# radiocosmology/draco

Measured on AMD Instinct MI355X. Metric: m-modes/sec through MModeTransform+DirtyMapMaker (128-feed, 256-freq), higher is better.
Workload: dtype f64 accumulate; B stored complex128; FFT complex64 (as the reference); 1 GPU; cfg3: 128-feed (379 stacked baselines), 256 freq per GPU (256 in the job), 1024 RA, lmax=mmax=512: MModeTransform.process + DirtyMapMaker.process through the task classes (131328 (m,f) solves + alm2map to nside=256 IQUV maps per GPU and day); parallelism=freq-sharded x1, weak scaling (no collective in the timed region)

## Files before the change

### draco_amd/csrc/sht.hip

```cpp
#include "sht_common.h"
#include "sht_legendre.h"
#include "sht_rings.h"

namespace {

int get_geom(dmm_ctx* ctx, int nside, int lmax, int mmax, ShtGeom* out) {
  const int64_t key = ((int64_t)nside << 40) | ((int64_t)lmax << 20) | (int64_t)mmax;
  auto it = ctx->sht.find(key);
  const int nring = 4 * nside - 1;
  const size_t nd = (size_t)3 * nring + (mmax + 1);
  const size_t bytes = nd * sizeof(double) + (size_t)nring * sizeof(int64_t) + (size_t)nring * sizeof(int);
  const size_t coef_ofs = (bytes + 63) / 64 * 64;
  const size_t coef_rows = (size_t)coef_row0(mmax + 1, lmax);
  int blue_rmax = 0;
  std::vector<int64_t> bf_off(1, 0);
  int64_t bf_total = 0;
  for (int ir = 1; ir < nside && blue_len(ir) <= kMaxBlue; ++ir) {
    bf_off.push_back(bf_total);
    bf_total += blue_len(ir);
    blue_rmax = ir;
  }
  const size_t bfo_ofs = coef_ofs + coef_rows * sizeof(Coef);
  const size_t bf_ofs = (bfo_ofs + bf_off.size() * sizeof(int64_t) + 63) / 64 * 64;
  const size_t phase_ofs = (bf_ofs + (size_t)bf_total * sizeof(double2) + 63) / 64 * 64;
// ... 86 lines not shown
  unsigned char* gb = static_cast<unsigned char*>(g.block);
  g.coef = reinterpret_cast<double*>(gb + coef_ofs);
  g.bf_off = reinterpret_cast<int64_t*>(gb + bfo_ofs);
  g.bfilt = reinterpret_cast<double2*>(gb + bf_ofs);
  g.blue_rmax = blue_rmax;
  g.phase = reinterpret_cast<double2*>(gb + phase_ofs);
  g.tw = reinterpret_cast<double2*>(gb + tw_ofs);
  g.tw_len = tw_len;
  g.chirp = reinterpret_cast<double2*>(gb + chirp_ofs);
  *out = g;
  return DMM_OK;
}

int check_args(const char* who, dmm_ctx* ctx, const void* a, const void* b, int nfreq, int npol, int lmax, int mmax,
               int nside) {
  DMM_REQUIRE(ctx && a && b, "%s: NULL argument", who);
  DMM_REQUIRE(nfreq >= 1 && lmax >= 0 && mmax >= 0 && mmax <= lmax, "%s: bad sizes nfreq=%d lmax=%d mmax=%d", who, nfreq, lmax, mmax);
  DMM_REQUIRE(npol == 1 || npol == 4, "%s: npol must be 1 or 4 (got %d)", who, npol);
  DMM_REQUIRE(nside >= 1 && (nside & (nside - 1)) == 0 && nside <= 8192, "%s: nside must be a power of two (got %d)", who, nside);
  return DMM_OK;
}

size_t chunk_freqs(int nfreq, int npol, int nring, int mmax) {
  const size_t per_f = (size_t)npol * nring * (mmax + 1) * sizeof(double2);
  size_t nf = ((size_t)1 << 30) / per_f;
  if (nf < 1) nf = 1;
  if (nf > (size_t)nfreq) nf = nfreq;
  const size_t nchunk = ((size_t)nfreq + nf - 1) / nf;
  return ((size_t)nfreq + nchunk - 1) / nchunk;
}

struct ClassLaunch {
  RingClass rc;
  int nblock;
  int nphi_max;
  bool blue;
};

std::vector<ClassLaunch> ring_classes(const ShtGeom& g) {
  std::vector<ClassLaunch> out;
  ClassLaunch b;
  b.rc.belt = 1;
  b.rc.r_lo = b.rc.r_hi = 0;
  b.rc.M = 4 * g.nside;
  b.rc.logM = 0;
  while ((1 << b.rc.logM) < b.rc.M) ++b.rc.logM;
  b.nblock = 2 * g.nside + 1;
  b.nphi_max = 4 * g.nside;
  b.blue = false;
  out.push_back(b);
  for (int ir = 1; ir < g.nside;) {
    const int M = blue_len(ir);
    int hi = ir;
    while (hi + 1 < g.nside && blue_len(hi + 1) == M) ++hi;
    ClassLaunch c;
    c.rc.belt = 0;
    c.rc.r_lo = ir;
    c.rc.r_hi = hi;
    c.rc.M = M;
    c.rc.logM = 0;
    while ((1 << c.rc.logM) < M) ++c.rc.logM;
    c.nblock = 2 * (hi - ir + 1);
    c.nphi_max = 4 * hi;
    c.blue = true;
    out.push_back(c);
    ir = hi + 1;
  }
  return out;
}

size_t ring_fft_lds(const ShtGeom& g, const ClassLaunch& c, int nrow, int force_direct, bool synth = false) {
  if (force_direct) return 0;
  if (c.blue && c.rc.r_hi > g.blue_rmax) return 0;
  const size_t rot = synth && c.blue && 4 * c.rc.r_lo < g.mmax + 1 ? (size_t)nrow * 2 * (g.mmax + 1) : 0;
  const size_t lds = ((size_t)nrow * (c.rc.M + 1) + c.rc.M / 2 + (c.blue ? c.nphi_max : 0) + rot) * sizeof(double2);
  return lds <= 160 * 1024 ? lds : 0;
}

template <typename K>
int launch_ring(K kern, dim3 grid, int threads, size_t lds, hipStream_t st, const RingParams& rp, const RingClass& rc) {
  if (lds > 160 * 1024) return dmm_set_error(DMM_E_UNSUPPORTED, "SHT ring stage needs %zu bytes of LDS (nside too large)", lds);
  DMM_HIP(hipFuncSetAttribute((const void*)kern, hipFuncAttributeMaxDynamicSharedMemorySize, (int)lds));
  hipLaunchKernelGGL(kern, grid, dim3(threads), lds, st, rp, rc);
  DMM_HIP(hipGetLastError());
  return DMM_OK;
}

template <int NPOL>
int synth_chunk(dmm_ctx* ctx, const ShtGeom& g, const double2* alm, int n_m, int nf, double2* b, double* map) {
  LegParams lp;
  lp.g = g;
  lp.nf = nf;
  lp.npol = NPOL;
  lp.n_m = n_m;
  lp.alm = alm;
  lp.b = b;
  lp.m_identity = (ctx->opt_sht_variant & 32) ? 1 : 0;
  if (NPOL == 4 && !(ctx->opt_sht_variant & 8)) {
    const int npair = (g.nring + 1) / 2;
    const int nrc = (npair + kThreads - 1) / kThreads;
#ifdef LEG_STAMPS
    static unsigned long long* stamps_d = nullptr;
    const size_t nst = (size_t)(g.mmax + 1) * nrc * ((nf + 2 * kLegF - 1) / (2 * kLegF)) * 4 * 8;
    if (!stamps_d) (void)hipMalloc((void**)&stamps_d, 64 << 20);
    (void)hipMemsetAsync(stamps_d, 0, nst * 8, ctx->stream);
    lp.stamps = stamps_d;
#endif
    const int nx = g.mmax + 1;
    const int64_t col_bytes = (int64_t)4 * n_m * (g.lmax + 1) * (int64_t)sizeof(double2);
    const bool fits8 = 2 * kLegF * col_bytes < ((int64_t)1 << 32), fits4 = kLegF * col_bytes < ((int64_t)1 << 32);
    if ((ctx->opt_sht_variant & 64) || ctx->opt_sht_synth_form == 1 || !fits4) {
      const int nz = (nf + kLegF - 1) / kLegF;
      hipLaunchKernelGGL(k_leg_synth_mfma, dim3(nx, nrc, nz), dim3(kThreads), 0, ctx->stream, lp);
    } else if ((ctx->opt_sht_variant & 128) || !fits8) {
      const int nz = (nf + kLegF - 1) / kLegF;
      hipLaunchKernelGGL(k_leg_synth_mfma2<1>, dim3(nx, nrc, nz), dim3(kThreads), 0, ctx->stream, lp);
    } else {
      const int nz = (nf + 2 * kLegF - 1) / (2 * kLegF);
      hipLaunchKernelGGL(k_leg_synth_mfma2<2>, dim3(nx, nrc, nz), dim3(kThreads), 0, ctx->stream, lp);
    }
  } else
  switch (ctx->opt_sht_variant & 3) {
    case 1: hipLaunchKernelGGL((k_leg_synth<NPOL, 1, 1>), dim3(g.mmax + 1, nf), dim3(kThreads), 0, ctx->stream, lp); break;
    case 2: hipLaunchKernelGGL((k_leg_synth<NPOL, 2, 1>), dim3(g.mmax + 1, nf), dim3(kThreads), 0, ctx->stream, lp); break;
    case 3: hipLaunchKernelGGL((k_leg_synth<NPOL, 1, 6>), dim3(g.mmax + 1, nf), dim3(kThreads), 0, ctx->stream, lp); break;
    default: hipLaunchKernelGGL((k_leg_synth<NPOL, 2, 4>), dim3(g.mmax + 1, nf), dim3(kThreads), 0, ctx->stream, lp); break;
  }
  DMM_HIP(hipGetLastError());
  RingParams rp;
  rp.g = g;
  rp.nf = nf;
  rp.npol = NPOL;
  rp.b = b;
  rp.map = map;
  rp.map_ref = nullptr;
  rp.radix8 = (ctx->opt_sht_variant & 2048) ? 0 : 1;
  rp.npix = 12LL * g.nside * g.nside;
  constexpr int NROWS = NPOL == 4 ? 2 : 1;
  const int force_direct = ctx->opt_sht_variant & 4;
  for (const ClassLaunch& c : ring_classes(g)) {
    const size_t lds2 = ring_fft_lds(g, c, NROWS, force_direct, true), lds1 = ring_fft_lds(g, c, 1, force_direct, true);
    int rc;
    if (lds1 == 0) {
      rc = launch_ring(k_ring_synth<NPOL>, dim3(c.nblock, nf), kThreads, (size_t)NPOL * (g.mmax + 1) * sizeof(double2), ctx->stream, rp, c.rc);
    } else if (NROWS == 2 && lds2 != 0 && lds2 <= 80 * 1024) {
      rc = c.blue ? launch_ring(k_ring_synth_fft<NPOL, NROWS, true>, dim3(c.nblock, nf), kFftThreads, lds2, ctx->stream, rp, c.rc)
                  : launch_ring(k_ring_synth_fft<NPOL, NROWS, false>, dim3(c.nblock, nf), kFftThreads, lds2, ctx->stream, rp, c.rc);
    } else {
      rc = c.blue ? launch_ring(k_ring_synth_fft<NPOL, 1, true>, dim3(c.nblock, nf, NROWS), kFftThreads, lds1, ctx->stream, rp, c.rc)
                  : launch_ring(k_ring_synth_fft<NPOL, 1, false>, dim3(c.nblock, nf, NROWS), kFftThreads, lds1, ctx->stream, rp, c.rc);
    }
    if (rc) return rc;
  }
  return DMM_OK;
}

template <int NPOL>
int anal_chunk(dmm_ctx* ctx, const ShtGeom& g, const double* map, int n_m, int nf, double2* b, double2* alm, int accumulate,
               const double* map_ref = nullptr) {
  RingParams rp;
  rp.g = g;
  rp.nf = nf;
  rp.npol = NPOL;
  rp.b = b;
  rp.map = const_cast<double*>(map);
  rp.map_ref = map_ref;
  rp.radix8 = (ctx->opt_sht_variant & 2048) ? 0 : 1;
  rp.npix = 12LL * g.nside * g.nside;
  constexpr int NROWS = NPOL == 4 ? 2 : 1;
  const int force_direct = ctx->opt_sht_variant & 4;
  for (const ClassLaunch& c : ring_classes(g)) {
    const size_t lds2 = ring_fft_lds(g, c, NROWS, force_direct), lds1 = ring_fft_lds(g, c, 1, force_direct);
    int rc;
    if (lds1 == 0) {
      rc = launch_ring(k_ring_anal<NPOL>, dim3(c.nblock, nf), kThreads, (size_t)NPOL * c.nphi_max * sizeof(double), ctx->stream, rp, c.rc);
    } else if (NROWS == 2 && lds2 != 0 && lds2 <= 80 * 1024) {
      rc = c.blue ? launch_ring(k_ring_anal_fft<NPOL, NROWS, true>, dim3(c.nblock, nf), kFftThreads, lds2, ctx->stream, rp, c.rc)
                  : launch_ring(k_ring_anal_fft<NPOL, NROWS, false>, dim3(c.nblock, nf), kFftThreads, lds2, ctx->stream, rp, c.rc);
    } else {
      rc = c.blue ? launch_ring(k_ring_anal_fft<NPOL, 1, true>, dim3(c.nblock, nf, NROWS), kFftThreads, lds1, ctx->stream, rp, c.rc)
                  : launch_ring(k_ring_anal_fft<NPOL, 1, false>, dim3(c.nblock, nf, NROWS), kFftThreads, lds1, ctx->stream, rp, c.rc);
    }
    if (rc) return rc;
  }
  LegAnalParams lp;
  lp.g = g;
  lp.nf = nf;
  lp.npol = NPOL;
  lp.n_m = n_m;
  lp.b = b;
  lp.alm = alm;
// ... 8 lines not shown
    return DMM_OK;
  }
  constexpr int NV = NPOL == 4 ? 8 : 2;
  const size_t lds2 = (size_t)(g.lmax + 1) * NV * sizeof(double) + (size_t)2 * (kThreads / 64) * kAnalBatch * NV * sizeof(double);
  DMM_HIP(hipFuncSetAttribute((const void*)k_leg_anal<NPOL>, hipFuncAttributeMaxDynamicSharedMemorySize, (int)lds2));
  hipLaunchKernelGGL(k_leg_anal<NPOL>, dim3(g.mmax + 1, nf), dim3(kThreads), lds2, ctx->stream, lp);
  DMM_HIP(hipGetLastError());
  return DMM_OK;
}

}

extern "C" {

int dmm_alm2map(dmm_ctx* ctx, const void* alm, int nfreq, int npol, int lmax, int mmax, int nside, double* map) {
  int rc = check_args("dmm_alm2map", ctx, alm, map, nfreq, npol, lmax, mmax, nside);
  if (rc) return rc;
  DMM_HIP(hipSetDevice(ctx->device));
  ShtGeom g;
  rc = get_geom(ctx, nside, lmax, mmax, &g);
  if (rc) return rc;
  const size_t nfc = chunk_freqs(nfreq, npol, g.nring, mmax);
  void* scratch = nullptr;
  rc = dmm_get_scratch(ctx, nfc * npol * g.nring * (size_t)(mmax + 1) * sizeof(double2), &scratch);
  if (rc) return rc;
  const int64_t npix = 12LL * nside * nside;
  const int n_m = mmax + 1;
  for (int f0 = 0; f0 < nfreq; f0 += (int)nfc) {
    const int nf = (int)((size_t)(nfreq - f0) < nfc ? (size_t)(nfreq - f0) : nfc);
    const double2* a = (const double2*)alm + (int64_t)f0 * npol * n_m * (lmax + 1);
    double* mp = map + (int64_t)f0 * npol * npix;
    rc = npol == 4 ? synth_chunk<4>(ctx, g, a, n_m, nf, (double2*)scratch, mp) : synth_chunk<1>(ctx, g, a, n_m, nf, (double2*)scratch, mp);
    if (rc) return rc;
  }
  return DMM_OK;
}

int dmm_map2alm(dmm_ctx* ctx, const double* map, int nfreq, int npol, int lmax, int mmax, int nside, int niter,
                void* alm) {
  int rc = check_args("dmm_map2alm", ctx, map, alm, nfreq, npol, lmax, mmax, nside);
  if (rc) return rc;
  DMM_REQUIRE(niter >= 0 && niter <= 64, "dmm_map2alm: niter=%d out of range", niter);
  if ((size_t)npol * 4 * nside * sizeof(double) > 150 * 1024)
    return dmm_set_error(DMM_E_UNSUPPORTED, "dmm_map2alm: nside=%d too large for the in-LDS ring stage", nside);
  DMM_HIP(hipSetDevice(ctx->device));
  ShtGeom g;
  rc = get_geom(ctx, nside, lmax, mmax, &g);
  if (rc) return rc;
  const int64_t npix = 12LL * nside * nside;
  size_t nfc = chunk_freqs(nfreq, npol, g.nring, mmax);
  const size_t b_bytes = nfc * npol * g.nring * (size_t)(mmax + 1) * sizeof(double2);
  const size_t r_bytes = niter > 0 ? nfc * npol * (size_t)npix * sizeof(double) : 0;
  void* scratch = nullptr;
  rc = dmm_get_scratch(ctx, b_bytes + r_bytes, &scratch);
  if (rc) return rc;
  double2* b = (double2*)scratch;
  double* resid = (double*)((unsigned char*)scratch + b_bytes);
  const int n_m = mmax + 1;
  for (int f0 = 0; f0 < nfreq; f0 += (int)nfc) {
    const int nf = (int)((size_t)(nfreq - f0) < nfc ? (size_t)(nfreq - f0) : nfc);
    double2* a = (double2*)alm + (int64_t)f0 * npol * n_m * (lmax + 1);
    const double* mp = map + (int64_t)f0 * npol * npix;
    rc = npol == 4 ? anal_chunk<4>(ctx, g, mp, n_m, nf, b, a, 0) : anal_chunk<1>(ctx, g, mp, n_m, nf, b, a, 0);
    if (rc) return rc;
    for (int it = 0; it < niter; ++it) {
      rc = npol == 4 ? synth_chunk<4>(ctx, g, a, n_m, nf, b, resid) : synth_chunk<1>(ctx, g, a, n_m, nf, b, resid);
      if (rc) return rc;
      rc = npol == 4 ? anal_chunk<4>(ctx, g, resid, n_m, nf, b, a, 1, mp) : anal_chunk<1>(ctx, g, resid, n_m, nf, b, a, 1, mp);
      if (rc) return rc;
    }
  }
  return DMM_OK;
}

// ... 2 lines not shown
```

### draco_amd/csrc/sht_common.h

```cpp
#pragma once
#include <math.h>

#include <vector>

#include "dmm_internal.h"
#include "fft_lds.h"

namespace {


constexpr int kThreads = 256;
constexpr double kBig = 0x1p+740, kSmallStep = 0x1p-800;

struct ShtGeom {
  int nside, lmax, mmax, nring;
  double* z;
  double* sth;
  double* phi0;
  int* nphi;
  int64_t* start;
  double* lfac;
  double* coef;
  double2* bfilt;
  int64_t* bf_off;
  int blue_rmax;
  double2* phase;
  double2* tw;
  int tw_len;
  double2* chirp;
  void* block;
};

__host__ __device__ __forceinline__ int64_t coef_row0(int m, int lmax) {
  return (int64_t)m * (lmax + 1) - (int64_t)m * (m - 1) / 2;
}

struct LegParams {
  ShtGeom g;
  int nf;
  int npol;
  int n_m;
  const double2* alm;
  double2* b;
  int m_identity;
#ifdef LEG_STAMPS
  unsigned long long* stamps;
#endif
};

struct Coef {
  double ra, rb;
  double c1, c2;
  double cd, c3;
  double c4, pad;
};

typedef const __attribute__((address_space(4))) double* kptr;

__device__ __forceinline__ Coef load_coef(kptr c) {
  Coef q;
  q.ra = c[0];
  q.rb = c[1];
  q.c1 = c[2];
  q.c2 = c[3];
  q.cd = c[4];
  q.c3 = c[5];
  q.c4 = c[6];
// ... 45 lines not shown
```

### draco_amd/csrc/sht_legendre.h

```cpp
#pragma once
#include "sht_common.h"

namespace {

__device__ __forceinline__ int leg_m_of_block(int b, int n_m, int variant_identity) {
  if (variant_identity) return b;
  const int q = b >> 6, r = b & 63;
  if (q * 64 + 64 > n_m) return b;
  return q * 64 + (r & 7) * 8 + (r >> 3);
}

template <int NPOL, int NR, int MINW>
__global__ __launch_bounds__(kThreads, MINW) void k_leg_synth(LegParams p) {
  const int m = blockIdx.x, f = blockIdx.y;
  const int lmax = p.g.lmax, nl = lmax - m + 1;
  const kptr coef = (kptr)p.g.coef + 8 * coef_row0(m, lmax);
  kptr a[NPOL];
#pragma unroll
  for (int q = 0; q < NPOL; ++q)
    a[q] = (kptr)(p.alm + (((int64_t)f * NPOL + q) * p.n_m + m) * (lmax + 1) + m);

  const int nring = p.g.nring, npair = (nring + 1) / 2;
  const double lfac_m = p.g.lfac[m];
  const int64_t mstride = p.g.mmax + 1;
  struct Ring {
    double x, inv_s2, xs2, lam, lam_prev;
    int nsc;
    double2 Ts, Ta, Vs, Va, Qs, Qa, Us, Ua;
  };
  for (int r0 = 0; r0 < npair; r0 += NR * kThreads) {
    Ring R[NR];
#pragma unroll
    for (int t = 0; t < NR; ++t) {
// ... 62 lines not shown
      if (NPOL == 4) {
        o.aE = load_c(a[NPOL > 1 ? 1 : 0] + 2 * kc);
        o.aB = load_c(a[NPOL > 1 ? 2 : 0] + 2 * kc);
        o.aV = load_c(a[NPOL > 1 ? 3 : 0] + 2 * kc);
      }
      return o;
    };
    Ops cur = fetch(0);
    for (int k = 0; k < nl; k += 2) {
      Ops nxt = fetch(k + 1);
#pragma unroll
      for (int t = 0; t < NR; ++t) step(R[t], cur.q, cur.aT, cur.aE, cur.aB, cur.aV, k == 0, true);
      if (k + 1 >= nl) break;
      cur = fetch(k + 2);
#pragma unroll
      for (int t = 0; t < NR; ++t) step(R[t], nxt.q, nxt.aT, nxt.aE, nxt.aB, nxt.aV, false, false);
    }
#pragma unroll
    for (int t = 0; t < NR; ++t) {
      const int r = r0 + t * kThreads + threadIdx.x;
      if (r >= npair) continue;
      const int rs = nring - 1 - r;
      const Ring& g = R[t];
      auto put = [&](int pol, int ring, double2 s, double2 an, double sgn) {
        p.b[(((int64_t)f * NPOL + pol) * nring + ring) * mstride + m] = make_double2(s.x + sgn * an.x, s.y + sgn * an.y);
      };
      put(0, r, g.Ts, g.Ta, 1.0);
      if (rs != r) put(0, rs, g.Ts, g.Ta, -1.0);
      if (NPOL == 4) {
        put(1, r, g.Qs, g.Qa, 1.0);
        put(2, r, g.Us, g.Ua, 1.0);
        put(3, r, g.Vs, g.Va, 1.0);
        if (rs != r) {
          put(1, rs, g.Qs, g.Qa, -1.0);
          put(2, rs, g.Us, g.Ua, -1.0);
          put(3, rs, g.Vs, g.Va, -1.0);
        }
      }
    }
  }
}

constexpr int kLegL = 8, kLegF = 4, kLegPitch = 72;

__device__ __forceinline__ void leg_synth_mfma_body(const LegParams& p, int bx, int by, int bz) {
  typedef double v4d __attribute__((ext_vector_type(4)));
  __shared__ double slab[kThreads / 64][3][kLegL][kLegPitch];
  const int m = leg_m_of_block(bx, p.g.mmax + 1, p.m_identity), rc = by, f0 = bz * kLegF;
  const int lmax = p.g.lmax, nl = lmax - m + 1;
  const int lane = threadIdx.x & 63, wave = threadIdx.x >> 6;
  const int nring = p.g.nring, npair = (nring + 1) / 2;
  const int64_t mstride = p.g.mmax + 1;
  double(*sl)[kLegL][kLegPitch] = slab[wave];

  const int r = rc * kThreads + threadIdx.x;
  double x = 0.0, inv_s2 = 0.0, xs2 = 0.0, lam = 0.0, lam_prev = 0.0;
  int nsc = -1;
  if (r < npair) {
    const double sth = p.g.sth[r];
    x = p.g.z[r];
    inv_s2 = 1.0 / (sth * sth);
    xs2 = x * inv_s2;
    if (!ring_skips_m(m, lmax, sth)) lam_start(p.g.lfac[m], m, sth, lam, nsc);
  }
  const bool wave_live = __any(nsc >= 0);

  const int li = lane & 15, kq = lane >> 4;
  const int col = li, fi = col >> 2, c = col & 3, f = f0 + fi;
  const bool fok = f < p.nf;
  auto colptr = [&](int pol, int comp) {
    return reinterpret_cast<const double*>(p.alm + (((int64_t)(fok ? f : 0) * 4 + pol) * p.n_m + m) * (lmax + 1) + m) + comp;
// ... 65 lines not shown
        sl[1][kk][lane] = F1;
        sl[2][kk][lane] = F2;
      }
      cv = cv_next;
#pragma unroll
      for (int par = 0; par < 2; ++par) {
        const bool ok = fok && c0 + 2 * kq + par < nl;
        const double bTV[2] = {ok ? rTV[0] : 0.0, ok ? rTV[1] : 0.0};
        const double b1[2] = {ok ? -r1[0] : 0.0, ok ? -r1[1] : 0.0};
        const double b2[2] = {ok ? s2 * r2[0] : 0.0, ok ? s2 * r2[1] : 0.0};
#pragma unroll
        for (int t = 0; t < 4; ++t) {
          const double aL = sl[0][2 * kq + par][16 * t + li];
          const double a1 = sl[1][2 * kq + par][16 * t + li];
          const double a2 = sl[2][2 * kq + par][16 * t + li];
          acc[t][par] = __builtin_amdgcn_mfma_f64_16x16x4f64(aL, bTV[par], acc[t][par], 0, 0, 0);
          acc[t][2 + par] = __builtin_amdgcn_mfma_f64_16x16x4f64(a1, b1[par], acc[t][2 + par], 0, 0, 0);
          acc[t][3 - par] = __builtin_amdgcn_mfma_f64_16x16x4f64(a2, b2[par], acc[t][3 - par], 0, 0, 0);
        }
      }
    }
  }
  if (!fok) return;
  double* bout = reinterpret_cast<double*>(p.b);
  const int comp = c & 1;
#pragma unroll
  for (int t = 0; t < 4; ++t)
#pragma unroll
    for (int reg = 0; reg < 4; ++reg) {
      const int rr = rc * kThreads + wave * 64 + 16 * t + kq + 4 * reg;
      if (rr >= npair) continue;
      const int rs = nring - 1 - rr;
#pragma unroll
      for (int g = 0; g < 2; ++g) {
        const int pol = g == 0 ? (c < 2 ? 0 : 3) : (c < 2 ? 1 : 2);
        const double sy = acc[t][2 * g][reg], an = acc[t][2 * g + 1][reg];
        bout[((((int64_t)f * 4 + pol) * nring + rr) * mstride + m) * 2 + comp] = sy + an;
        if (rs != rr) bout[((((int64_t)f * 4 + pol) * nring + rs) * mstride + m) * 2 + comp] = sy - an;
      }
    }
}

__global__ __launch_bounds__(kThreads, 2) void k_leg_synth_mfma(LegParams p) { leg_synth_mfma_body(p, blockIdx.x, blockIdx.y, blockIdx.z); }


constexpr int kLeg2Rows = kLegL + 1;
#ifndef PIPE_HINT
#define PIPE_HINT 1
#endif

template <int NFG>
__device__ __forceinline__ void leg_synth_mfma2_body(const LegParams& p, int bx, int by, int bz, int ny) {
  typedef double v4d __attribute__((ext_vector_type(4)));
  __shared__ double slab[kThreads / 64][2][kLeg2Rows][kLegPitch];
  __shared__ double ringf[kThreads / 64][2][64];
  const int m = leg_m_of_block(bx, p.g.mmax + 1, p.m_identity), rc = by, f0 = bz * (kLegF * NFG);
  const int lmax = p.g.lmax, nl = lmax - m + 1;
  const int lane = threadIdx.x & 63, wave = threadIdx.x >> 6;
  const int nring = p.g.nring, npair = (nring + 1) / 2;
  const int64_t mstride = p.g.mmax + 1;
  double(*sl)[kLeg2Rows][kLegPitch] = slab[wave];
#ifdef LEG_STAMPS
  unsigned long long st[6];
  auto stamp = [&](int i) {
    unsigned long long t;
    __builtin_amdgcn_sched_barrier(0);
    asm volatile("s_memrealtime %0\n\ts_waitcnt lgkmcnt(0)" : "=s"(t)::"memory");
    __builtin_amdgcn_sched_barrier(0);
    st[i] = t;
  };
  stamp(0);
#define LEG_STAMP(i) stamp(i)
#else
#define LEG_STAMP(i)
#endif

  const int NW = ny * (kThreads / 64), W = rc * (kThreads / 64) + wave;
  const int r = 16 * (W + (lane >> 4) * NW) + (lane & 15);
  double x = 0.0, lam = 0.0, lam_prev = 0.0;
// ... 164 lines not shown
      prep_load(nb, 0, 0);
      cvr = cvr_next;
      finish_ops(ops_next, c0n, ragged);
      ops = ops_next;
    };
    LEG_STAMP(2);
    int ch = 0;
    for (; ch + 1 < nchunk && __any(nsc > 0); ++ch) body(ch, true);
    LEG_STAMP(3);
    for (; ch + 1 < nchunk; ++ch) body(ch, false);
    {
      const int b = ch & 1;
      prep_build(0, ops);
#pragma unroll
      for (int g = 0; g < kLegL; ++g) {
        if (g + 1 < kLegL) prep_load(b, (g + 1) & 3, (g + 1) >> 2);
        issue(g & 3, g >> 2, ops);
        if (g + 1 < kLegL) prep_build((g + 1) >> 2, ops);
        __builtin_amdgcn_sched_barrier(0);
      }
    }
  }
  LEG_STAMP(4);
  double* bout = reinterpret_cast<double*>(p.b);
  const int comp = c & 1;
#pragma unroll
  for (int h = 0; h < NFG; ++h) {
    if (!fok[h]) continue;
    const int f = fq[h];
#pragma unroll
    for (int t = 0; t < 4; ++t)
#pragma unroll
      for (int reg = 0; reg < 4; ++reg) {
        const int rr = 16 * (W + t * NW) + kq + 4 * reg;
        if (rr >= npair) continue;
        const int rs = nring - 1 - rr;
#pragma unroll
        for (int g = 0; g < 2; ++g) {
          const int pol = g == 0 ? (c < 2 ? 0 : 3) : (c < 2 ? 1 : 2);
          const double sy = acc[h][t][2 * g][reg], an = acc[h][t][2 * g + 1][reg];
          bout[((((int64_t)f * 4 + pol) * nring + rr) * mstride + m) * 2 + comp] = sy + an;
          if (rs != rr) bout[((((int64_t)f * 4 + pol) * nring + rs) * mstride + m) * 2 + comp] = sy - an;
        }
      }
  }
#ifdef LEG_STAMPS
  stamp(5);
  if (p.stamps && lane == 0) {
    unsigned hw;
    asm volatile("s_getreg_b32 %0, hwreg(HW_REG_HW_ID)" : "=s"(hw));
    unsigned xcc;
    asm volatile("s_getreg_b32 %0, hwreg(HW_REG_XCC_ID)" : "=s"(xcc));
    unsigned long long* o = p.stamps + 8 * ((((size_t)blockIdx.z * gridDim.y + blockIdx.y) * gridDim.x + blockIdx.x) * 4 + wave);
    for (int i = 0; i < 6; ++i) o[i] = wave_live ? st[i] : (i == 0 || i == 5 ? st[i] : st[0]);
    o[6] = ((unsigned long long)xcc << 32) | hw;
    o[7] = m;
  }
#endif
}

template <int NFG>
__global__ __launch_bounds__(kThreads, 3 - NFG) void k_leg_synth_mfma2(LegParams p) {
  leg_synth_mfma2_body<NFG>(p, blockIdx.x, blockIdx.y, blockIdx.z, gridDim.y);
}

struct LegAnalParams {
  ShtGeom g;
  int nf, npol, n_m;
  const double2* b;
  double2* alm;
  int accumulate;
  int m_identity;
};

template <int NV>
__device__ __forceinline__ double wave_reduce_scatter(double (&v)[NV], int lane) {
  static_assert(NV == 8 || NV == 2, "NV");
  double z;
  if (NV == 8) {
    double w[4], u[2];
    const bool up5 = lane & 32, up4 = lane & 16, up3 = lane & 8;
#pragma unroll
    for (int i = 0; i < 4; ++i) w[i] = (up5 ? v[4 + i] : v[i]) + __shfl_xor(up5 ? v[i] : v[4 + i], 32, 64);
#pragma unroll
    for (int i = 0; i < 2; ++i) u[i] = (up4 ? w[2 + i] : w[i]) + __shfl_xor(up4 ? w[i] : w[2 + i], 16, 64);
    z = (up3 ? u[1] : u[0]) + __shfl_xor(up3 ? u[0] : u[1], 8, 64);
// ... 342 lines not shown
```

### draco_amd/csrc/sht_rings.h

```cpp
#pragma once
#include "sht_common.h"

namespace {

struct RingParams {
  ShtGeom g;
  int nf, npol;
  double2* b;
  double* map;
  int64_t npix;
  const double* map_ref;
  int radix8;
};

struct RingClass {
  int belt;
  int r_lo, r_hi;
  int M, logM;
};
constexpr int kMinBlue = 256, kMaxBlue = 4096;

__host__ __device__ __forceinline__ int blue_len(int ir) {
  int M = kMinBlue;
  while (M < 8 * ir - 1) M <<= 1;
  return M;
}

__device__ __forceinline__ int class_ring(const RingClass& rc, const ShtGeom& g, int i) {
  if (rc.belt) return g.nside - 1 + i;
  const int ir = rc.r_lo + (i >> 1);
  return (i & 1) ? g.nring - ir : ir - 1;
}

template <int NPOL>
__global__ __launch_bounds__(kThreads) void k_ring_synth(RingParams p, RingClass rc) {
  extern __shared__ __align__(16) unsigned char smem[];
  double2* c = reinterpret_cast<double2*>(smem);
  const int ring = class_ring(rc, p.g, blockIdx.x);
  const int f = blockIdx.y;
  const int nm = p.g.mmax + 1;
  const double phi0 = p.g.phi0[ring];
  const int nphi = p.g.nphi[ring];
  for (int idx = threadIdx.x; idx < NPOL * nm; idx += kThreads) {
    const int pol = idx / nm, m = idx - pol * nm;
    const double2 v = p.b[(((int64_t)f * NPOL + pol) * p.g.nring + ring) * nm + m];
    double sn, cs;
    sincos((double)m * phi0, &sn, &cs);
    const double fac = m == 0 ? 1.0 : 2.0;
    c[idx] = make_double2(fac * (v.x * cs - v.y * sn), fac * (v.x * sn + v.y * cs));
  }
  __syncthreads();
  const int64_t base = p.g.start[ring];
  for (int j = threadIdx.x; j < nphi; j += kThreads) {
    double sn, cs;
    sincospi(2.0 * (double)j / (double)nphi, &sn, &cs);
    double pr = 1.0, pi_ = 0.0;
    double acc[NPOL];
#pragma unroll
    for (int q = 0; q < NPOL; ++q) acc[q] = 0.0;
    for (int m = 0; m < nm; ++m) {
#pragma unroll
      for (int q = 0; q < NPOL; ++q) {
        const double2 cm = c[q * nm + m];
        acc[q] = fma(cm.x, pr, fma(-cm.y, pi_, acc[q]));
      }
      const double nr = pr * cs - pi_ * sn;
      pi_ = fma(pr, sn, pi_ * cs);
      pr = nr;
// ... 64 lines not shown
template <int NROW, bool BLUE>
__device__ __forceinline__ void ring_dft(const RingLds& l, const double2* bfilt, int M, int logM, bool radix8 = false) {
  const int P = M + 1;
  if (radix8) dmm_fft::fft_dif8<double, kFftThreads>(l.buf, l.tw, NROW, M, logM, P);
  else dmm_fft::fft_dif<double, kFftThreads>(l.buf, l.tw, NROW, M, logM, P);
  if (BLUE) {
    for (int idx = threadIdx.x; idx < NROW * M; idx += kFftThreads) {
      const int r = idx / M, k = idx - r * M;
      const double2 fk = bfilt[k];
      l.buf[r * P + k] = dmm_fft::cmul<double>(l.buf[r * P + k], {fk.x, fk.y});
    }
    __syncthreads();
    if (radix8) dmm_fft::fft_dit8<double, true, kFftThreads>(l.buf, l.tw, NROW, M, logM, P);
    else dmm_fft::fft_dit<double, true, kFftThreads>(l.buf, l.tw, NROW, M, logM, P);
  }
}

template <bool BLUE>
__device__ __forceinline__ dmm_fft::C<double> ring_dft_at(const RingLds& l, int r, int k, int M, int logM) {
  if (BLUE) return dmm_fft::cmul<double>(l.buf[r * (M + 1) + k], l.chirp[k]);
  return l.buf[r * (M + 1) + dmm_fft::bitrev(k, logM)];
}

template <int NPOL, int NROW, bool BLUE>
__global__ __launch_bounds__(kFftThreads) void k_ring_synth_fft(RingParams p, RingClass rc) {
  using dmm_fft::C;
  extern __shared__ __align__(16) unsigned char smem[];
  const int rb = blockIdx.z * NROW;
  const int ring = class_ring(rc, p.g, blockIdx.x), f = blockIdx.y;
  const int n = p.g.nphi[ring], M = rc.M, P = M + 1;
  const RingLds l = ring_lds<NROW, BLUE>(smem, p.g, n, M);
  if (BLUE) __syncthreads();
  const int nm = p.g.mmax + 1;
  const double2* phase = p.g.phase + (int64_t)ring * nm;
  const double2 *browa[NROW], *browb[NROW];
#pragma unroll
  for (int r = 0; r < NROW; ++r) {
    browa[r] = p.b + (((int64_t)f * NPOL + (NPOL == 4 ? 2 * (r + rb) : 0)) * p.g.nring + ring) * nm;
    browb[r] = p.b + (((int64_t)f * NPOL + (NPOL == 4 ? 2 * (r + rb) + 1 : 0)) * p.g.nring + ring) * nm;
  }
  const bool aliased = n < nm;
  C<double>* rot = l.chirp + (BLUE ? 4 * rc.r_hi : 0);
  if (aliased) {
    for (int m = threadIdx.x; m < nm; m += kFftThreads) {
      const double2 ph = phase[m];
      const double cs = ph.x, sn = ph.y;
#pragma unroll
      for (int r = 0; r < NROW; ++r) {
        const double2 va = browa[r][m];
        C<double> a = {va.x * cs - va.y * sn, va.x * sn + va.y * cs}, b = {0.0, 0.0};
        if (NPOL == 4) {
          const double2 vb = browb[r][m];
          b = {vb.x * cs - vb.y * sn, vb.x * sn + vb.y * cs};
        }
        if (m == 0) a.y = b.y = 0.0;
        rot[(r * 2 + 0) * nm + m] = a;
        rot[(r * 2 + 1) * nm + m] = b;
      }
    }
    __syncthreads();
  }
  for (int k = threadIdx.x; k < M; k += kFftThreads) {
    double zr[NROW], zi[NROW];
#pragma unroll
    for (int r = 0; r < NROW; ++r) zr[r] = zi[r] = 0.0;
    if (k < n && aliased) {
      for (int m = k; m < nm; m += n) {
#pragma unroll
        for (int r = 0; r < NROW; ++r) {
          const C<double> a = rot[(r * 2 + 0) * nm + m], b = rot[(r * 2 + 1) * nm + m];
          zr[r] += a.x - b.y;
          zi[r] += a.y + b.x;
        }
      }
      for (int m = (k == 0 ? n : n - k); m < nm; m += n) {
#pragma unroll
        for (int r = 0; r < NROW; ++r) {
          const C<double> a = rot[(r * 2 + 0) * nm + m], b = rot[(r * 2 + 1) * nm + m];
          zr[r] += a.x + b.y;
          zi[r] += b.x - a.y;
        }
      }
    } else if (k < n) {
      for (int m = k; m < nm; m += n) {
        const double2 ph = phase[m];
        const double cs = ph.x, sn = ph.y;
#pragma unroll
        for (int r = 0; r < NROW; ++r) {
          const double2 va = browa[r][m];
          double ar = va.x * cs - va.y * sn, ai = va.x * sn + va.y * cs;
          double br = 0.0, bi = 0.0;
          if (NPOL == 4) {
            const double2 vb = browb[r][m];
            br = vb.x * cs - vb.y * sn;
            bi = vb.x * sn + vb.y * cs;
          }
          if (m == 0) ai = bi = 0.0;
          zr[r] += ar - bi;
          zi[r] += ai + br;
        }
      }
      for (int m = (k == 0 ? n : n - k); m < nm; m += n) {
        const double2 ph = phase[m];
        const double cs = ph.x, sn = ph.y;
#pragma unroll
        for (int r = 0; r < NROW; ++r) {
          const double2 va = browa[r][m];
          const double ar = va.x * cs - va.y * sn, ai = va.x * sn + va.y * cs;
          double br = 0.0, bi = 0.0;
          if (NPOL == 4) {
            const double2 vb = browb[r][m];
            br = vb.x * cs - vb.y * sn;
            bi = vb.x * sn + vb.y * cs;
          }
          zr[r] += ar + bi;
          zi[r] += br - ai;
        }
      }
    }
#pragma unroll
    for (int r = 0; r < NROW; ++r) {
      C<double> v = {zr[r], -zi[r]};
      if (BLUE && k < n) v = dmm_fft::cmul<double>(v, l.chirp[k]);
      l.buf[r * P + k] = v;
    }
  }
  __syncthreads();
  const double2* bfilt = BLUE ? p.g.bfilt + p.g.bf_off[rc.belt ? 0 : rc.r_lo + ((int)blockIdx.x >> 1)] : nullptr;
  ring_dft<NROW, BLUE>(l, bfilt, M, rc.logM, p.radix8 != 0);
  const int64_t base = p.g.start[ring];
  for (int j = threadIdx.x; j < n; j += kFftThreads) {
#pragma unroll
    for (int r = 0; r < NROW; ++r) {
      const C<double> y = ring_dft_at<BLUE>(l, r, j, M, rc.logM);
      p.map[((int64_t)f * NPOL + (NPOL == 4 ? 2 * (r + rb) : 0)) * p.npix + base + j] = y.x;
      if (NPOL == 4) p.map[((int64_t)f * NPOL + 2 * (r + rb) + 1) * p.npix + base + j] = -y.y;
    }
  }
}

template <int NPOL>
__global__ __launch_bounds__(kThreads) void k_ring_anal(RingParams p, RingClass rc) {
  extern __shared__ __align__(16) unsigned char smem[];
  double* px = reinterpret_cast<double*>(smem);
  const int ring = class_ring(rc, p.g, blockIdx.x), f = blockIdx.y;
  const int nm = p.g.mmax + 1;
  const double phi0 = p.g.phi0[ring];
  const int nphi = p.g.nphi[ring];
  const int64_t base = p.g.start[ring];
  for (int idx = threadIdx.x; idx < NPOL * nphi; idx += kThreads) {
    const int pol = idx / nphi, j = idx - pol * nphi;
    const int64_t pi = ((int64_t)f * NPOL + pol) * p.npix + base + j;
    px[idx] = p.map_ref ? p.map_ref[pi] - p.map[pi] : p.map[pi];
  }
  __syncthreads();
  const double w = 4.0 * M_PI / (double)p.npix;
  for (int m = threadIdx.x; m < nm; m += kThreads) {
    double sn, cs;
    sincospi(-2.0 * (double)(m % nphi) / (double)nphi, &sn, &cs);
// ... 105 lines not shown
```

Baseline: 2010 m-modes/s.

## Interleave synthesis scratch by frequency groups and batch ring FFTs across frequencies

Changes the Legendre-synthesis output buffer layout so four frequencies and paired polarizations sit interleaved per (ring, m), written as double2 vector stores. The ring synthesis FFT kernel now processes a group of frequencies per block, choosing the batch size from an LDS budget tier, and optionally stages all phase-rotated coefficients in LDS. The aim is coalesced wider stores and loads between the Legendre and ring stages and fewer blocks with better data reuse. It also drops the m-block swizzle and rounds chunk sizes to the group size, at the cost of more complex indexing and possibly lower occupancy from larger LDS use.

```diff
diff --git a/draco_amd/csrc/sht.hip b/draco_amd/csrc/sht.hip
--- a/draco_amd/csrc/sht.hip
+++ b/draco_amd/csrc/sht.hip
@@ -132,12 +132,19 @@
 }
 
 size_t chunk_freqs(int nfreq, int npol, int nring, int mmax) {
+  const size_t grp = npol == 4 ? kSynF : 1;
   const size_t per_f = (size_t)npol * nring * (mmax + 1) * sizeof(double2);
-  size_t nf = ((size_t)1 << 30) / per_f;
-  if (nf < 1) nf = 1;
+  size_t nf = ((size_t)1 << 30) / per_f / grp * grp;
+  if (nf < grp) nf = grp;
   if (nf > (size_t)nfreq) nf = nfreq;
   const size_t nchunk = ((size_t)nfreq + nf - 1) / nf;
-  return ((size_t)nfreq + nchunk - 1) / nchunk;
+  const size_t c = ((size_t)nfreq + nchunk - 1) / nchunk;
+  return c < (size_t)nfreq ? (c + grp - 1) / grp * grp : c;
+}
+
+size_t coef_scratch_bytes(size_t nfc, int npol, int nring, int mmax) {
+  const size_t nfs = npol == 4 ? (nfc + kSynF - 1) / kSynF * kSynF : nfc;
+  return nfs * npol * nring * (size_t)(mmax + 1) * sizeof(double2);
 }
 
 struct ClassLaunch {
@@ -179,11 +186,20 @@
   return out;
 }
 
-size_t ring_fft_lds(const ShtGeom& g, const ClassLaunch& c, int nrow, int force_direct, bool synth = false) {
+size_t ring_fft_lds(const ShtGeom& g, const ClassLaunch& c, int nrow, int force_direct) {
   if (force_direct) return 0;
   if (c.blue && c.rc.r_hi > g.blue_rmax) return 0;
-  const size_t rot = synth && c.blue && 4 * c.rc.r_lo < g.mmax + 1 ? (size_t)nrow * 2 * (g.mmax + 1) : 0;
-  const size_t lds = ((size_t)nrow * (c.rc.M + 1) + c.rc.M / 2 + (c.blue ? c.nphi_max : 0) + rot) * sizeof(double2);
+  const size_t lds = ((size_t)nrow * (c.rc.M + 1) + c.rc.M / 2 + (c.blue ? c.nphi_max : 0)) * sizeof(double2);
+  return lds <= 160 * 1024 ? lds : 0;
+}
+
+size_t ring_synth_lds(const ShtGeom& g, const ClassLaunch& c, int nb, bool stage_all, int force_direct) {
+  if (force_direct) return 0;
+  if (c.blue && c.rc.r_hi > g.blue_rmax) return 0;
+  const int nm = g.mmax + 1;
+  const bool staged = stage_all || 4 * (c.blue ? c.rc.r_lo : g.nside) < nm;
+  const size_t lds = ((size_t)nb * (c.rc.M + 1) + c.rc.M / 2 + (c.blue ? c.nphi_max : 0) + (staged ? (size_t)nb * 2 * nm : 0)) *
+                     sizeof(double2);
   return lds <= 160 * 1024 ? lds : 0;
 }
 
@@ -205,7 +221,6 @@
   lp.n_m = n_m;
   lp.alm = alm;
   lp.b = b;
-  lp.m_identity = (ctx->opt_sht_variant & 32) ? 1 : 0;
   if (NPOL == 4 && !(ctx->opt_sht_variant & 8)) {
     const int npair = (g.nring + 1) / 2;
     const int nrc = (npair + kThreads - 1) / kThreads;
@@ -246,19 +261,32 @@
   rp.map_ref = nullptr;
   rp.radix8 = (ctx->opt_sht_variant & 2048) ? 0 : 1;
   rp.npix = 12LL * g.nside * g.nside;
-  constexpr int NROWS = NPOL == 4 ? 2 : 1;
+  rp.stage_all = 0;
+  constexpr int KF = NPOL == 4 ? kSynF : 1;
+  const dim3 per_ring((nf + KF - 1) / KF, NPOL == 4 ? 2 : 1);
   const int force_direct = ctx->opt_sht_variant & 4;
   for (const ClassLaunch& c : ring_classes(g)) {
-    const size_t lds2 = ring_fft_lds(g, c, NROWS, force_direct, true), lds1 = ring_fft_lds(g, c, 1, force_direct, true);
+    int nb = 0;
+    size_t lds = 0;
+    rp.stage_all = 0;
+    for (int tier = 0; tier < 3 && nb == 0; ++tier)
+      for (int b = KF; b >= 1 && nb == 0; b >>= 1) {
+        const size_t l = ring_synth_lds(g, c, b, tier == 0, force_direct);
+        if (l != 0 && l <= (tier < 2 ? (size_t)80 * 1024 : (size_t)160 * 1024)) nb = b, lds = l, rp.stage_all = tier == 0;
+      }
+    const dim3 grid(c.nblock, per_ring.x, per_ring.y);
     int rc;
-    if (lds1 == 0) {
+    if (nb == 0) {
       rc = launch_ring(k_ring_synth<NPOL>, dim3(c.nblock, nf), kThreads, (size_t)NPOL * (g.mmax + 1) * sizeof(double2), ctx->stream, rp, c.rc);
-    } else if (NROWS == 2 && lds2 != 0 && lds2 <= 80 * 1024) {
-      rc = c.blue ? launch_ring(k_ring_synth_fft<NPOL, NROWS, true>, dim3(c.nblock, nf), kFftThreads, lds2, ctx->stream, rp, c.rc)
-                  : launch_ring(k_ring_synth_fft<NPOL, NROWS, false>, dim3(c.nblock, nf), kFftThreads, lds2, ctx->stream, rp, c.rc);
+    } else if (nb == 4) {
+      rc = c.blue ? launch_ring(k_ring_synth_fft<NPOL, NPOL == 4 ? 4 : 1, true>, grid, kFftThreads, lds, ctx->stream, rp, c.rc)
+                  : launch_ring(k_ring_synth_fft<NPOL, NPOL == 4 ? 4 : 1, false>, grid, kFftThreads, lds, ctx->stream, rp, c.rc);
+    } else if (nb == 2) {
+      rc = c.blue ? launch_ring(k_ring_synth_fft<NPOL, NPOL == 4 ? 2 : 1, true>, grid, kFftThreads, lds, ctx->stream, rp, c.rc)
+                  : launch_ring(k_ring_synth_fft<NPOL, NPOL == 4 ? 2 : 1, false>, grid, kFftThreads, lds, ctx->stream, rp, c.rc);
     } else {
-      rc = c.blue ? launch_ring(k_ring_synth_fft<NPOL, 1, true>, dim3(c.nblock, nf, NROWS), kFftThreads, lds1, ctx->stream, rp, c.rc)
-                  : launch_ring(k_ring_synth_fft<NPOL, 1, false>, dim3(c.nblock, nf, NROWS), kFftThreads, lds1, ctx->stream, rp, c.rc);
+      rc = c.blue ? launch_ring(k_ring_synth_fft<NPOL, 1, true>, grid, kFftThreads, lds, ctx->stream, rp, c.rc)
+                  : launch_ring(k_ring_synth_fft<NPOL, 1, false>, grid, kFftThreads, lds, ctx->stream, rp, c.rc);
     }
     if (rc) return rc;
   }
@@ -277,6 +305,7 @@
   rp.map_ref = map_ref;
   rp.radix8 = (ctx->opt_sht_variant & 2048) ? 0 : 1;
   rp.npix = 12LL * g.nside * g.nside;
+  rp.stage_all = 0;
   constexpr int NROWS = NPOL == 4 ? 2 : 1;
   const int force_direct = ctx->opt_sht_variant & 4;
   for (const ClassLaunch& c : ring_classes(g)) {
@@ -331,7 +360,7 @@
   if (rc) return rc;
   const size_t nfc = chunk_freqs(nfreq, npol, g.nring, mmax);
   void* scratch = nullptr;
-  rc = dmm_get_scratch(ctx, nfc * npol * g.nring * (size_t)(mmax + 1) * sizeof(double2), &scratch);
+  rc = dmm_get_scratch(ctx, coef_scratch_bytes(nfc, npol, g.nring, mmax), &scratch);
   if (rc) return rc;
   const int64_t npix = 12LL * nside * nside;
   const int n_m = mmax + 1;
@@ -358,7 +387,7 @@
   if (rc) return rc;
   const int64_t npix = 12LL * nside * nside;
   size_t nfc = chunk_freqs(nfreq, npol, g.nring, mmax);
-  const size_t b_bytes = nfc * npol * g.nring * (size_t)(mmax + 1) * sizeof(double2);
+  const size_t b_bytes = coef_scratch_bytes(nfc, npol, g.nring, mmax);
   const size_t r_bytes = niter > 0 ? nfc * npol * (size_t)npix * sizeof(double) : 0;
   void* scratch = nullptr;
   rc = dmm_get_scratch(ctx, b_bytes + r_bytes, &scratch);
diff --git a/draco_amd/csrc/sht_common.h b/draco_amd/csrc/sht_common.h
--- a/draco_amd/csrc/sht_common.h
+++ b/draco_amd/csrc/sht_common.h
@@ -11,6 +11,13 @@
 
 constexpr int kThreads = 256;
 constexpr double kBig = 0x1p+740, kSmallStep = 0x1p-800;
+
+constexpr int kSynF = 4;
+constexpr int kSynRow = kSynF * 4;
+__host__ __device__ __forceinline__ int64_t syn4_at(int f, int m, int ring, int r, int nring, int nm) {
+  return ((((int64_t)(f / kSynF) * 2 + r) * nring + ring) * nm + m) * kSynRow + 4 * (f % kSynF);
+}
+__host__ __device__ __forceinline__ int syn4_slot(int pol) { return pol == 1 || pol == 2 ? 1 : 0; }
 
 struct ShtGeom {
   int nside, lmax, mmax, nring;
@@ -42,7 +49,6 @@
   int n_m;
   const double2* alm;
   double2* b;
-  int m_identity;
 #ifdef LEG_STAMPS
   unsigned long long* stamps;
 #endif
diff --git a/draco_amd/csrc/sht_legendre.h b/draco_amd/csrc/sht_legendre.h
--- a/draco_amd/csrc/sht_legendre.h
+++ b/draco_amd/csrc/sht_legendre.h
@@ -2,13 +2,6 @@
 #include "sht_common.h"
 
 namespace {
-
-__device__ __forceinline__ int leg_m_of_block(int b, int n_m, int variant_identity) {
-  if (variant_identity) return b;
-  const int q = b >> 6, r = b & 63;
-  if (q * 64 + 64 > n_m) return b;
-  return q * 64 + (r & 7) * 8 + (r >> 3);
-}
 
 template <int NPOL, int NR, int MINW>
 __global__ __launch_bounds__(kThreads, MINW) void k_leg_synth(LegParams p) {
@@ -117,19 +110,22 @@
       if (r >= npair) continue;
       const int rs = nring - 1 - r;
       const Ring& g = R[t];
-      auto put = [&](int pol, int ring, double2 s, double2 an, double sgn) {
-        p.b[(((int64_t)f * NPOL + pol) * nring + ring) * mstride + m] = make_double2(s.x + sgn * an.x, s.y + sgn * an.y);
-      };
-      put(0, r, g.Ts, g.Ta, 1.0);
-      if (rs != r) put(0, rs, g.Ts, g.Ta, -1.0);
-      if (NPOL == 4) {
-        put(1, r, g.Qs, g.Qa, 1.0);
-        put(2, r, g.Us, g.Ua, 1.0);
-        put(3, r, g.Vs, g.Va, 1.0);
+      auto val = [&](double2 s, double2 an, double sgn) { return make_double2(s.x + sgn * an.x, s.y + sgn * an.y); };
+      if (NPOL == 1) {
+        p.b[((int64_t)f * nring + r) * mstride + m] = val(g.Ts, g.Ta, 1.0);
+        if (rs != r) p.b[((int64_t)f * nring + rs) * mstride + m] = val(g.Ts, g.Ta, -1.0);
+      } else {
+        double* bout = reinterpret_cast<double*>(p.b);
+        auto put = [&](int ring, int tr, double2 v0, double2 v1) {
+          double* q = bout + syn4_at(f, m, ring, tr, nring, (int)mstride);
+          *reinterpret_cast<double2*>(q) = make_double2(v0.x, v1.x);
+          *reinterpret_cast<double2*>(q + 2) = make_double2(v0.y, v1.y);
+        };
+        put(r, 0, val(g.Ts, g.Ta, 1.0), val(g.Qs, g.Qa, 1.0));
+        put(r, 1, val(g.Vs, g.Va, 1.0), val(g.Us, g.Ua, 1.0));
         if (rs != r) {
-          put(1, rs, g.Qs, g.Qa, -1.0);
-          put(2, rs, g.Us, g.Ua, -1.0);
-          put(3, rs, g.Vs, g.Va, -1.0);
+          put(rs, 0, val(g.Ts, g.Ta, -1.0), val(g.Qs, g.Qa, -1.0));
+          put(rs, 1, val(g.Vs, g.Va, -1.0), val(g.Us, g.Ua, -1.0));
         }
       }
     }
@@ -137,11 +133,12 @@
 }
 
 constexpr int kLegL = 8, kLegF = 4, kLegPitch = 72;
+static_assert(kLegF == kSynF, "a frequency group of the MFMA columns is one group of the synthesis scratch");
 
 __device__ __forceinline__ void leg_synth_mfma_body(const LegParams& p, int bx, int by, int bz) {
   typedef double v4d __attribute__((ext_vector_type(4)));
   __shared__ double slab[kThreads / 64][3][kLegL][kLegPitch];
-  const int m = leg_m_of_block(bx, p.g.mmax + 1, p.m_identity), rc = by, f0 = bz * kLegF;
+  const int m = bx, rc = by, f0 = bz * kLegF;
   const int lmax = p.g.lmax, nl = lmax - m + 1;
   const int lane = threadIdx.x & 63, wave = threadIdx.x >> 6;
   const int nring = p.g.nring, npair = (nring + 1) / 2;
@@ -253,8 +250,7 @@
     }
   }
   if (!fok) return;
-  double* bout = reinterpret_cast<double*>(p.b);
-  const int comp = c & 1;
+  double* bout = reinterpret_cast<double*>(p.b) + 2 * (c & 1);
 #pragma unroll
   for (int t = 0; t < 4; ++t)
 #pragma unroll
@@ -262,13 +258,9 @@
       const int rr = rc * kThreads + wave * 64 + 16 * t + kq + 4 * reg;
       if (rr >= npair) continue;
       const int rs = nring - 1 - rr;
-#pragma unroll
-      for (int g = 0; g < 2; ++g) {
-        const int pol = g == 0 ? (c < 2 ? 0 : 3) : (c < 2 ? 1 : 2);
-        const double sy = acc[t][2 * g][reg], an = acc[t][2 * g + 1][reg];
-        bout[((((int64_t)f * 4 + pol) * nring + rr) * mstride + m) * 2 + comp] = sy + an;
-        if (rs != rr) bout[((((int64_t)f * 4 + pol) * nring + rs) * mstride + m) * 2 + comp] = sy - an;
-      }
+      const double tv = acc[t][0][reg], tva = acc[t][1][reg], qu = acc[t][2][reg], qua = acc[t][3][reg];
+      *reinterpret_cast<double2*>(bout + syn4_at(f, m, rr, c >> 1, nring, (int)mstride)) = make_double2(tv + tva, qu + qua);
+      if (rs != rr) *reinterpret_cast<double2*>(bout + syn4_at(f, m, rs, c >> 1, nring, (int)mstride)) = make_double2(tv - tva, qu - qua);
     }
 }
 
@@ -285,7 +277,7 @@
   typedef double v4d __attribute__((ext_vector_type(4)));
   __shared__ double slab[kThreads / 64][2][kLeg2Rows][kLegPitch];
   __shared__ double ringf[kThreads / 64][2][64];
-  const int m = leg_m_of_block(bx, p.g.mmax + 1, p.m_identity), rc = by, f0 = bz * (kLegF * NFG);
+  const int m = bx, rc = by, f0 = bz * (kLegF * NFG);
   const int lmax = p.g.lmax, nl = lmax - m + 1;
   const int lane = threadIdx.x & 63, wave = threadIdx.x >> 6;
   const int nring = p.g.nring, npair = (nring + 1) / 2;
@@ -496,8 +488,7 @@
     }
   }
   LEG_STAMP(4);
-  double* bout = reinterpret_cast<double*>(p.b);
-  const int comp = c & 1;
+  double* bout = reinterpret_cast<double*>(p.b) + 2 * (c & 1);
 #pragma unroll
   for (int h = 0; h < NFG; ++h) {
     if (!fok[h]) continue;
@@ -509,13 +500,9 @@
         const int rr = 16 * (W + t * NW) + kq + 4 * reg;
         if (rr >= npair) continue;
         const int rs = nring - 1 - rr;
-#pragma unroll
-        for (int g = 0; g < 2; ++g) {
-          const int pol = g == 0 ? (c < 2 ? 0 : 3) : (c < 2 ? 1 : 2);
-          const double sy = acc[h][t][2 * g][reg], an = acc[h][t][2 * g + 1][reg];
-          bout[((((int64_t)f * 4 + pol) * nring + rr) * mstride + m) * 2 + comp] = sy + an;
-          if (rs != rr) bout[((((int64_t)f * 4 + pol) * nring + rs) * mstride + m) * 2 + comp] = sy - an;
-        }
+        const double tv = acc[h][t][0][reg], tva = acc[h][t][1][reg], qu = acc[h][t][2][reg], qua = acc[h][t][3][reg];
+        *reinterpret_cast<double2*>(bout + syn4_at(f, m, rr, c >> 1, nring, (int)mstride)) = make_double2(tv + tva, qu + qua);
+        if (rs != rr) *reinterpret_cast<double2*>(bout + syn4_at(f, m, rs, c >> 1, nring, (int)mstride)) = make_double2(tv - tva, qu - qua);
       }
   }
 #ifdef LEG_STAMPS
@@ -536,6 +523,13 @@
 template <int NFG>
 __global__ __launch_bounds__(kThreads, 3 - NFG) void k_leg_synth_mfma2(LegParams p) {
   leg_synth_mfma2_body<NFG>(p, blockIdx.x, blockIdx.y, blockIdx.z, gridDim.y);
+}
+
+__device__ __forceinline__ int leg_m_of_block(int b, int n_m, int variant_identity) {
+  if (variant_identity) return b;
+  const int q = b >> 6, r = b & 63;
+  if (q * 64 + 64 > n_m) return b;
+  return q * 64 + (r & 7) * 8 + (r >> 3);
 }
 
 struct LegAnalParams {
diff --git a/draco_amd/csrc/sht_rings.h b/draco_amd/csrc/sht_rings.h
--- a/draco_amd/csrc/sht_rings.h
+++ b/draco_amd/csrc/sht_rings.h
@@ -11,6 +11,7 @@
   int64_t npix;
   const double* map_ref;
   int radix8;
+  int stage_all;
 };
 
 struct RingClass {
@@ -43,7 +44,13 @@
   const int nphi = p.g.nphi[ring];
   for (int idx = threadIdx.x; idx < NPOL * nm; idx += kThreads) {
     const int pol = idx / nm, m = idx - pol * nm;
-    const double2 v = p.b[(((int64_t)f * NPOL + pol) * p.g.nring + ring) * nm + m];
+    double2 v;
+    if (NPOL == 1) {
+      v = p.b[((int64_t)f * p.g.nring + ring) * nm + m];
+    } else {
+      const double* q = reinterpret_cast<const double*>(p.b) + syn4_at(f, m, ring, pol >> 1, p.g.nring, nm) + syn4_slot(pol);
+      v = make_double2(q[0], q[2]);
+    }
     double sn, cs;
     sincos((double)m * phi0, &sn, &cs);
     const double fac = m == 0 ? 1.0 : 2.0;
@@ -154,119 +161,131 @@
   return l.buf[r * (M + 1) + dmm_fft::bitrev(k, logM)];
 }
 
-template <int NPOL, int NROW, bool BLUE>
+template <int NPOL, int NB, bool BLUE>
 __global__ __launch_bounds__(kFftThreads) void k_ring_synth_fft(RingParams p, RingClass rc) {
   using dmm_fft::C;
+  constexpr int KF = NPOL == 4 ? kSynF : 1;
+  static_assert(KF % NB == 0, "passes of NB transforms");
   extern __shared__ __align__(16) unsigned char smem[];
-  const int rb = blockIdx.z * NROW;
-  const int ring = class_ring(rc, p.g, blockIdx.x), f = blockIdx.y;
+  const int ring = class_ring(rc, p.g, blockIdx.x), r = NPOL == 4 ? (int)blockIdx.z : 0;
+  const int f0 = KF * blockIdx.y, nfb = min(KF, p.nf - f0);
   const int n = p.g.nphi[ring], M = rc.M, P = M + 1;
-  const RingLds l = ring_lds<NROW, BLUE>(smem, p.g, n, M);
+  const RingLds l = ring_lds<NB, BLUE>(smem, p.g, n, M);
   if (BLUE) __syncthreads();
   const int nm = p.g.mmax + 1;
   const double2* phase = p.g.phase + (int64_t)ring * nm;
-  const double2 *browa[NROW], *browb[NROW];
-#pragma unroll
-  for (int r = 0; r < NROW; ++r) {
-    browa[r] = p.b + (((int64_t)f * NPOL + (NPOL == 4 ? 2 * (r + rb) : 0)) * p.g.nring + ring) * nm;
-    browb[r] = p.b + (((int64_t)f * NPOL + (NPOL == 4 ? 2 * (r + rb) + 1 : 0)) * p.g.nring + ring) * nm;
-  }
-  const bool aliased = n < nm;
+  auto load = [&](int fi, int m, double2& va, double2& vb) {
+    if (NPOL == 1) {
+      va = p.b[((int64_t)(f0 + fi) * p.g.nring + ring) * nm + m];
+    } else {
+      const double* q = reinterpret_cast<const double*>(p.b) + syn4_at(f0 + fi, m, ring, r, p.g.nring, nm);
+      const double2 re = *reinterpret_cast<const double2*>(q), im = *reinterpret_cast<const double2*>(q + 2);
+      va = r == 0 ? make_double2(re.x, im.x) : make_double2(re.y, im.y);
+      vb = r == 0 ? make_double2(re.y, im.y) : make_double2(re.x, im.x);
+    }
+  };
+  const bool staged = p.stage_all || n < nm;
   C<double>* rot = l.chirp + (BLUE ? 4 * rc.r_hi : 0);
-  if (aliased) {
-    for (int m = threadIdx.x; m < nm; m += kFftThreads) {
-      const double2 ph = phase[m];
-      const double cs = ph.x, sn = ph.y;
-#pragma unroll
-      for (int r = 0; r < NROW; ++r) {
-        const double2 va = browa[r][m];
-        C<double> a = {va.x * cs - va.y * sn, va.x * sn + va.y * cs}, b = {0.0, 0.0};
-        if (NPOL == 4) {
-          const double2 vb = browb[r][m];
-          b = {vb.x * cs - vb.y * sn, vb.x * sn + vb.y * cs};
+  const double2* bfilt = BLUE ? p.g.bfilt + p.g.bf_off[rc.belt ? 0 : rc.r_lo + ((int)blockIdx.x >> 1)] : nullptr;
+  const int64_t base = p.g.start[ring];
+  for (int fb = 0; fb < nfb; fb += NB) {
+    if (fb > 0) __syncthreads();
+    if (staged) {
+      for (int q = threadIdx.x; q < NB * nm; q += kFftThreads) {
+        const int m = q / NB, j = q - m * NB;
+        C<double> a = {0.0, 0.0}, b = {0.0, 0.0};
+        if (fb + j < nfb) {
+          const double2 ph = phase[m];
+          const double cs = ph.x, sn = ph.y;
+          double2 va, vb;
+          load(fb + j, m, va, vb);
+          a = {va.x * cs - va.y * sn, va.x * sn + va.y * cs};
+          if (NPOL == 4) b = {vb.x * cs - vb.y * sn, vb.x * sn + vb.y * cs};
+          if (m == 0) a.y = b.y = 0.0;
         }
-        if (m == 0) a.y = b.y = 0.0;
-        rot[(r * 2 + 0) * nm + m] = a;
-        rot[(r * 2 + 1) * nm + m] = b;
+        rot[(j * 2 + 0) * nm + m] = a;
+        rot[(j * 2 + 1) * nm + m] = b;
+      }
+      __syncthreads();
+    }
+    for (int k = threadIdx.x; k < M; k += kFftThreads) {
+      double zr[NB], zi[NB];
+#pragma unroll
+      for (int j = 0; j < NB; ++j) zr[j] = zi[j] = 0.0;
+      if (k < n && staged) {
+        for (int m = k; m < nm; m += n) {
+#pragma unroll
+          for (int j = 0; j < NB; ++j) {
+            const C<double> a = rot[(j * 2 + 0) * nm + m], b = rot[(j * 2 + 1) * nm + m];
+            zr[j] += a.x - b.y;
+            zi[j] += a.y + b.x;
+          }
+        }
+        for (int m = (k == 0 ? n : n - k); m < nm; m += n) {
+#pragma unroll
+          for (int j = 0; j < NB; ++j) {
+            const C<double> a = rot[(j * 2 + 0) * nm + m], b = rot[(j * 2 + 1) * nm + m];
+            zr[j] += a.x + b.y;
+            zi[j] += b.x - a.y;
+          }
+        }
+      } else if (k < n) {
+        for (int m = k; m < nm; m += n) {
+          const double2 ph = phase[m];
+          const double cs = ph.x, sn = ph.y;
+#pragma unroll
+          for (int j = 0; j < NB; ++j) {
+            if (fb + j >= nfb) continue;
+            double2 va, vb;
+            load(fb + j, m, va, vb);
+            double ar = va.x * cs - va.y * sn, ai = va.x * sn + va.y * cs;
+            double br = 0.0, bi = 0.0;
+            if (NPOL == 4) {
+              br = vb.x * cs - vb.y * sn;
+              bi = vb.x * sn + vb.y * cs;
+            }
+            if (m == 0) ai = bi = 0.0;
+            zr[j] += ar - bi;
+            zi[j] += ai + br;
+          }
+        }
+        for (int m = (k == 0 ? n : n - k); m < nm; m += n) {
+          const double2 ph = phase[m];
+          const double cs = ph.x, sn = ph.y;
+#pragma unroll
+          for (int j = 0; j < NB; ++j) {
+            if (fb + j >= nfb) continue;
+            double2 va, vb;
+            load(fb + j, m, va, vb);
+            const double ar = va.x * cs - va.y * sn, ai = va.x * sn + va.y * cs;
+            double br = 0.0, bi = 0.0;
+            if (NPOL == 4) {
+              br = vb.x * cs - vb.y * sn;
+              bi = vb.x * sn + vb.y * cs;
+            }
+            zr[j] += ar + bi;
+            zi[j] += br - ai;
+          }
+        }
+      }
+#pragma unroll
+      for (int j = 0; j < NB; ++j) {
+        C<double> v = {zr[j], -zi[j]};
+        if (BLUE && k < n) v = dmm_fft::cmul<double>(v, l.chirp[k]);
+        l.buf[j * P + k] = v;
       }
     }
     __syncthreads();
-  }
-  for (int k = threadIdx.x; k < M; k += kFftThreads) {
-    double zr[NROW], zi[NROW];
-#pragma unroll
-    for (int r = 0; r < NROW; ++r) zr[r] = zi[r] = 0.0;
-    if (k < n && aliased) {
-      for (int m = k; m < nm; m += n) {
-#pragma unroll
-        for (int r = 0; r < NROW; ++r) {
-          const C<double> a = rot[(r * 2 + 0) * nm + m], b = rot[(r * 2 + 1) * nm + m];
-          zr[r] += a.x - b.y;
-          zi[r] += a.y + b.x;
-        }
-      }
-      for (int m = (k == 0 ? n : n - k); m < nm; m += n) {
-#pragma unroll
-        for (int r = 0; r < NROW; ++r) {
-          const C<double> a = rot[(r * 2 + 0) * nm + m], b = rot[(r * 2 + 1) * nm + m];
-          zr[r] += a.x + b.y;
-          zi[r] += b.x - a.y;
-        }
-      }
-    } else if (k < n) {
-      for (int m = k; m < nm; m += n) {
-        const double2 ph = phase[m];
-        const double cs = ph.x, sn = ph.y;
-#pragma unroll
-        for (int r = 0; r < NROW; ++r) {
-          const double2 va = browa[r][m];
-          double ar = va.x * cs - va.y * sn, ai = va.x * sn + va.y * cs;
-          double br = 0.0, bi = 0.0;
-          if (NPOL == 4) {
-            const double2 vb = browb[r][m];
-            br = vb.x * cs - vb.y * sn;
-            bi = vb.x * sn + vb.y * cs;
-          }
-          if (m == 0) ai = bi = 0.0;
-          zr[r] += ar - bi;
-          zi[r] += ai + br;
-        }
-      }
-      for (int m = (k == 0 ? n : n - k); m < nm; m += n) {
-        const double2 ph = phase[m];
-        const double cs = ph.x, sn = ph.y;
-#pragma unroll
-        for (int r = 0; r < NROW; ++r) {
-          const double2 va = browa[r][m];
-          const double ar = va.x * cs - va.y * sn, ai = va.x * sn + va.y * cs;
-          double br = 0.0, bi = 0.0;
-          if (NPOL == 4) {
-            const double2 vb = browb[r][m];
-            br = vb.x * cs - vb.y * sn;
-            bi = vb.x * sn + vb.y * cs;
-          }
-          zr[r] += ar + bi;
-          zi[r] += br - ai;
-        }
-      }
-    }
-#pragma unroll
-    for (int r = 0; r < NROW; ++r) {
-      C<double> v = {zr[r], -zi[r]};
-      if (BLUE && k < n) v = dmm_fft::cmul<double>(v, l.chirp[k]);
-      l.buf[r * P + k] = v;
-    }
-  }
-  __syncthreads();
-  const double2* bfilt = BLUE ? p.g.bfilt + p.g.bf_off[rc.belt ? 0 : rc.r_lo + ((int)blockIdx.x >> 1)] : nullptr;
-  ring_dft<NROW, BLUE>(l, bfilt, M, rc.logM, p.radix8 != 0);
-  const int64_t base = p.g.start[ring];
-  for (int j = threadIdx.x; j < n; j += kFftThreads) {
-#pragma unroll
-    for (int r = 0; r < NROW; ++r) {
-      const C<double> y = ring_dft_at<BLUE>(l, r, j, M, rc.logM);
-      p.map[((int64_t)f * NPOL + (NPOL == 4 ? 2 * (r + rb) : 0)) * p.npix + base + j] = y.x;
-      if (NPOL == 4) p.map[((int64_t)f * NPOL + 2 * (r + rb) + 1) * p.npix + base + j] = -y.y;
+    ring_dft<NB, BLUE>(l, bfilt, M, rc.logM, p.radix8 != 0);
+    for (int j = threadIdx.x; j < n; j += kFftThreads) {
+#pragma unroll
+      for (int jj = 0; jj < NB; ++jj) {
+        if (fb + jj >= nfb) continue;
+        const int64_t f = f0 + fb + jj;
+        const C<double> y = ring_dft_at<BLUE>(l, jj, j, M, rc.logM);
+        p.map[(f * NPOL + 2 * r) * p.npix + base + j] = y.x;
+        if (NPOL == 4) p.map[(f * NPOL + 2 * r + 1) * p.npix + base + j] = -y.y;
+      }
     }
   }
 }
```

Result: faster. 2054 m-modes/s (median of 6 runs) (+2.2%).
